# planck-epoch/unet-image-segmentation

Measured on AMD Instinct MI355X. Metric: images/sec (train step, 256x256x3), higher is better.
Workload: dtype f32; 1 GPU; configs[1]: 256x256x3 binary U-Net train step (fwd + dice_loss + bwd + AdamW + MeanIoU(2) update, dropout 0.2); network=U_NET separable-conv, filters 64-128-256-512, bneck 1024, global_batch=16, per_gpu_batch=16, seq_len=65536, parallelism=dp1, batchnorm=per-replica

## Files before the change

unet-image-segmentation_amd/csrc/gemm_wgrad.hip:

```cpp
#include "dispatch.h"
#include "gemm.h"

namespace unet {
namespace {

template <int BP, int BQ, int AMODE, bool ADROP, int BMODE, bool BDROP>
__global__ __launch_bounds__(256) void gemm_wgrad_kernel(WgradArgs g) {
    constexpr int LDA = BP + 4, LDB = BQ + 4;
    constexpr int TM = BP / 64, TN = BQ / 64;
    constexpr int AR = BP / 16, BR = BQ / 16;
    constexpr int AS = 256 / BP, BS = 256 / BQ;
    __shared__ float As[2][BK][LDA];
    __shared__ float Bs[2][BK][LDB];

    const int tid = threadIdx.x, lane = tid & 63, wave = tid >> 6;
    const int wp = wave >> 1, wq = wave & 1;
    const int lo = lane & 31, hi = lane >> 5;
    const int ntp = (g.P + BP - 1) / BP;
    const int p0 = (blockIdx.x % ntp) * BP;
    const int q0 = (blockIdx.x / ntp) * BQ;
    const int64_t mb = (int64_t)blockIdx.y * g.mslice;
    const int64_t me = mb + g.mslice < g.M ? mb + g.mslice : g.M;

    const int ap = tid % BP, amm = tid / BP;
    const int p = p0 + ap;
    const bool pv = p < g.P;
    float asc = 1.f, ash = 0.f;
    int poff = p;
    if constexpr (AMODE == W_BNRELU) {
        if (pv) {
            asc = g.a.sc0[p];
            ash = g.a.sh0[p];
        }
    }
    if constexpr (AMODE == W_UNSHUFFLE) {
        const int ab = p / g.uf;
        const int co = p - ab * g.uf;
        poff = (ab >> 1) * (2 * g.uW * g.uf) + (ab & 1) * g.uf + co;
    }
    const int bq = tid % BQ, bmm = tid / BQ;
    const int q = q0 + bq;
    const bool qv = q < g.Q;
    float bsc = 1.f, bsh = 0.f;
    if constexpr (BMODE == W_BNRELU) {
        if (qv) {
            bsc = g.b.sc0[q];
            bsh = g.b.sh0[q];
        }
    }

    float ra[AR], rb[BR];
    auto load_stage = [&](int64_t k0) {
#pragma unroll
        for (int r = 0; r < AR; ++r) {
            const int64_t m = k0 + amm + AS * r;
            float v = 0.f;
            if (pv && m < me) {
                if constexpr (AMODE == W_UNSHUFFLE) {
                    const int64_t hw = (int64_t)g.uH * g.uW;
                    const int n = (int)(m / hw);
                    const int rem = (int)(m - n * hw);
                    const int i = rem / g.uW, j = rem - (rem / g.uW) * g.uW;
                    v = g.a.src0[(int64_t)((n * 2 * g.uH + 2 * i) * 2 * g.uW + 2 * j) * g.uf + poff];
                } else {
                    v = g.a.src0[m * g.a.c0 + p];
                    if constexpr (AMODE == W_BNRELU) v = bnrelu(v, asc, ash);
                    if constexpr (ADROP) v *= drop_mult(g.a.seed, (uint64_t)m * g.a.C + p, g.a.rate, g.a.inv_keep);
                }
            }
            ra[r] = v;
        }
#pragma unroll
        for (int r = 0; r < BR; ++r) {
            const int64_t m = k0 + bmm + BS * r;
            float v = 0.f;
            if (qv && m < me) {
                v = g.b.src0[m * g.b.c0 + q];
                if constexpr (BMODE == W_BNRELU) v = bnrelu(v, bsc, bsh);
                if constexpr (BDROP) v *= drop_mult(g.b.seed, (uint64_t)m * g.b.C + q, g.b.rate, g.b.inv_keep);
            }
            rb[r] = v;
        }
    };
    auto store_stage = [&](int buf) {
#pragma unroll
        for (int r = 0; r < AR; ++r) As[buf][amm + AS * r][ap] = ra[r];
#pragma unroll
        for (int r = 0; r < BR; ++r) Bs[buf][bmm + BS * r][bq] = rb[r];
    };

    floatx16 acc[TM][TN];
#pragma unroll
    for (int tm = 0; tm < TM; ++tm)
#pragma unroll
        for (int tn = 0; tn < TN; ++tn)
#pragma unroll
            for (int r = 0; r < 16; ++r) acc[tm][tn][r] = 0.f;

    const int nk = (int)((me - mb + BK - 1) / BK);
    if (nk > 0) {
        load_stage(mb);
        store_stage(0);
    }
    __syncthreads();
    for (int kt = 0; kt < nk; ++kt) {
        const int buf = kt & 1;
        if (kt + 1 < nk) load_stage(mb + (int64_t)(kt + 1) * BK);
#pragma unroll
        for (int kk = 0; kk < BK / 2; ++kk) {
            float av[TM], bv[TN];
#pragma unroll
            for (int tm = 0; tm < TM; ++tm) av[tm] = As[buf][2 * kk + hi][wp * (BP / 2) + tm * 32 + lo];
#pragma unroll
            for (int tn = 0; tn < TN; ++tn) bv[tn] = Bs[buf][2 * kk + hi][wq * (BQ / 2) + tn * 32 + lo];
#pragma unroll
            for (int tm = 0; tm < TM; ++tm)
#pragma unroll
                for (int tn = 0; tn < TN; ++tn)
                    acc[tm][tn] = __builtin_amdgcn_mfma_f32_32x32x2f32(av[tm], bv[tn], acc[tm][tn], 0, 0, 0);
        }
        if (kt + 1 < nk) store_stage(buf ^ 1);
        __syncthreads();
    }
    float* slab = g.slab + (int64_t)blockIdx.y * g.P * g.Q;
#pragma unroll
    for (int tm = 0; tm < TM; ++tm)
#pragma unroll
        for (int tn = 0; tn < TN; ++tn) {
            const int qq = q0 + wq * (BQ / 2) + tn * 32 + lo;
            if (qq >= g.Q) continue;
#pragma unroll
            for (int r = 0; r < 16; ++r) {
                const int pp = p0 + wp * (BP / 2) + tm * 32 + acc_row(r, hi);
                if (pp < g.P) slab[(int64_t)pp * g.Q + qq] = acc[tm][tn][r];
            }
        }
}

template <int BP, int BQ, int AMODE, bool ADROP, int BMODE, bool BDROP>
__global__ __launch_bounds__(256, 1) void gemm_wgrad_vec(WgradArgs g) {
    constexpr int LDA = BP + 4, LDB = BQ + 4;
    constexpr int TM = BP / 64, TN = BQ / 64;
    constexpr int PQ = BP / 4, QQ = BQ / 4;
    constexpr int AR = BK * PQ / 256, BR = BK * QQ / 256;
    constexpr int AS = 256 / PQ, BS = 256 / QQ;
    __shared__ __attribute__((aligned(16))) char smem[4 * 2 * BK * (LDA + LDB)];
    float (*As)[BK * LDA] = reinterpret_cast<float (*)[BK * LDA]>(smem);
    float (*Bs)[BK * LDB] = reinterpret_cast<float (*)[BK * LDB]>(smem + 4 * 2 * BK * LDA);

    const int tid = threadIdx.x, lane = tid & 63, wave = tid >> 6;
    const int wp = wave >> 1, wq = wave & 1;
    const int lo = lane & 31, hi = lane >> 5;
    const int ntp = (g.P + BP - 1) / BP;
    int tile, slice;
    xcd_group_order_sx(gridDim.x, gridDim.y, tile, slice);
    const int p0 = (tile % ntp) * BP;
    const int q0 = (tile / ntp) * BQ;
    const int mb = (int)(slice * g.mslice);
    const int me = (int)((mb + g.mslice) < g.M ? (mb + g.mslice) : g.M);

    const int apq = tid % PQ, amm = tid / PQ;
    const int p = p0 + 4 * apq;
    const bool pv = p < g.P;
    float4 asc = f4(1.f), ash = f4(0.f);
    int poff = p;
    if constexpr (AMODE == W_BNRELU) {
        if (pv) {
            asc = ld4(g.a.sc0 + p);
            ash = ld4(g.a.sh0 + p);
        }
    }
    if constexpr (AMODE == W_UNSHUFFLE) {
        const int ab = p / g.uf;
        const int co = p - ab * g.uf;
        poff = (ab >> 1) * (2 * g.uW * g.uf) + (ab & 1) * g.uf + co;
    }
    const int bqq = tid % QQ, bmm = tid / QQ;
    const int q = q0 + 4 * bqq;
    const bool qv = q < g.Q;
    float4 bsc = f4(1.f), bsh = f4(0.f), bmu = f4(0.f), bp_ = f4(0.f), bq_ = f4(0.f);
    if constexpr (BMODE == W_BNRELU || BMODE == W_BNBWD) {
        if (qv) {
            bsc = ld4(g.b.sc0 + q);
            bsh = ld4(g.b.sh0 + q);
        }
    }
    if constexpr (BMODE == W_BNBWD) {
        if (qv) {
            bmu = ld4(g.bcoef + q);
            bp_ = ld4(g.bcoef + g.Q + q);
            bq_ = ld4(g.bcoef + 2 * g.Q + q);
        }
    }

    float4 ra[AR], rb[BR];
    int ur[AMODE == W_UNSHUFFLE ? AR : 1], uj[AMODE == W_UNSHUFFLE ? AR : 1];
    if constexpr (AMODE == W_UNSHUFFLE) {
#pragma unroll
        for (int r = 0; r < AR; ++r) {
            const int m = mb + amm + AS * r;
            ur[r] = m / g.uW;
            uj[r] = m - ur[r] * g.uW;
        }
    }
    auto load_stage = [&](int k0) {
#pragma unroll
        for (int r = 0; r < AR; ++r) {
            const int m = k0 + amm + AS * r;
            float4 v = f4(0.f);
            if (pv && m < me) {
                if constexpr (AMODE == W_UNSHUFFLE) {
                    v = ld4(g.a.src0 + (4 * ur[r] * g.uW + 2 * uj[r]) * g.uf + poff);
                } else {
                    v = ld4(g.a.src0 + (int64_t)m * g.a.c0 + p);
                    if constexpr (AMODE == W_BNRELU) v = bnrelu4(v, asc, ash);
                    if constexpr (ADROP) {
                        const uint64_t i = (uint64_t)m * g.a.C + p;
                        v = mul4(v, drop_mult4(g.a.seed, i, g.a.rate, g.a.inv_keep));
                    }
                }
            }
            ra[r] = v;
        }
#pragma unroll
        for (int r = 0; r < BR; ++r) {
            const int m = k0 + bmm + BS * r;
            float4 v = f4(0.f);
            if (qv && m < me) {
                v = ld4(g.b.src0 + (int64_t)m * g.b.c0 + q);
                if constexpr (BMODE == W_BNRELU) v = bnrelu4(v, bsc, bsh);
                if constexpr (BMODE == W_BNBWD)
                    bn_bwd_dz4(v, ld4(g.bz + (int64_t)m * g.b.c0 + q), bsc, bsh, bmu, bp_, bq_);
                if constexpr (BDROP) {
                    const uint64_t i = (uint64_t)m * g.b.C + q;
                    v = mul4(v, drop_mult4(g.b.seed, i, g.b.rate, g.b.inv_keep));
                }
            }
            rb[r] = v;
        }
        if constexpr (AMODE == W_UNSHUFFLE) {
#pragma unroll
            for (int r = 0; r < AR; ++r) {
                uj[r] += BK;
                while (uj[r] >= g.uW) {
                    uj[r] -= g.uW;
                    ++ur[r];
                }
            }
        }
    };
    const bool csum_on = g.colpart != nullptr && tile < ntp;
    float4 csum = f4(0.f);
    auto store_stage = [&](int buf) {
#pragma unroll
        for (int r = 0; r < AR; ++r) *reinterpret_cast<float4*>(&As[buf][(amm + AS * r) * LDA + 4 * apq]) = ra[r];
#pragma unroll
        for (int r = 0; r < BR; ++r) *reinterpret_cast<float4*>(&Bs[buf][(bmm + BS * r) * LDB + 4 * bqq]) = rb[r];
        if (csum_on) {
#pragma unroll
            for (int r = 0; r < AR; ++r) csum = add4(csum, ra[r]);
        }
    };

    floatx16 acc[TM][TN];
#pragma unroll
    for (int tm = 0; tm < TM; ++tm)
#pragma unroll
        for (int tn = 0; tn < TN; ++tn)
#pragma unroll
            for (int r = 0; r < 16; ++r) acc[tm][tn][r] = 0.f;

    const int nk = (me - mb + BK - 1) / BK;
    if (nk > 0) {
        load_stage(mb);
        store_stage(0);
    }
    __syncthreads();
    for (int kt = 0; kt < nk; ++kt) {
        const int buf = kt & 1;
        if (kt + 1 < nk) load_stage(mb + (kt + 1) * BK);
#pragma unroll
        for (int kk = 0; kk < BK / 2; ++kk) {
            float av[TM], bv[TN];
#pragma unroll
            for (int tm = 0; tm < TM; ++tm) av[tm] = As[buf][(2 * kk + hi) * LDA + wp * (BP / 2) + tm * 32 + lo];
#pragma unroll
            for (int tn = 0; tn < TN; ++tn) bv[tn] = Bs[buf][(2 * kk + hi) * LDB + wq * (BQ / 2) + tn * 32 + lo];
#pragma unroll
            for (int tm = 0; tm < TM; ++tm)
#pragma unroll
                for (int tn = 0; tn < TN; ++tn)
                    acc[tm][tn] = __builtin_amdgcn_mfma_f32_32x32x2f32(av[tm], bv[tn], acc[tm][tn], 0, 0, 0);
        }
        if (kt + 1 < nk) store_stage(buf ^ 1);
        __syncthreads();
    }
    if (csum_on) {
        float4* T = reinterpret_cast<float4*>(&As[0][0]);
        T[tid] = csum;
        __syncthreads();
        if (tid < PQ && pv) {
            float4 t = T[tid];
            for (int j = 1; j < AS; ++j) t = add4(t, T[j * PQ + tid]);
            st4(g.colpart + (int64_t)slice * g.P + p, t);
        }
    }
    float* slab = g.slab + (int64_t)slice * g.P * g.Q;
#pragma unroll
    for (int tm = 0; tm < TM; ++tm)
#pragma unroll
        for (int tn = 0; tn < TN; ++tn) {
            const int qq = q0 + wq * (BQ / 2) + tn * 32 + lo;
            if (qq >= g.Q) continue;
#pragma unroll
            for (int r = 0; r < 16; ++r) {
                const int pp = p0 + wp * (BP / 2) + tm * 32 + acc_row(r, hi);
                if (pp < g.P) slab[(int64_t)pp * g.Q + qq] = acc[tm][tn][r];
            }
        }
}

template <int AMODE, bool ADROP, int BMODE, bool BDROP>
void launch_wgrad_t(const WgradArgs& a, const WgradPlan& w, hipStream_t st) {
    dim3 grid((unsigned)w.tiles, (unsigned)w.S);
    const unsigned pad = (unsigned)lab_knob("UNET_WGRAD_LDSPAD", 0);
    const bool vec = a.P % 4 == 0 && a.Q % 4 == 0 && (AMODE != W_UNSHUFFLE || a.uf % 4 == 0) &&
                     (AMODE == W_UNSHUFFLE || a.a.c0 % 4 == 0) && a.b.c0 % 4 == 0 &&
                     ((uintptr_t)a.a.src0 | (uintptr_t)a.b.src0) % 16 == 0;
    const bool vk = vec || BMODE == W_BNBWD;
    with_int<128, 64>(w.bp, [&](auto BP) {
        with_int<128, 64>(w.bq, [&](auto BQ) {
            if (vk) gemm_wgrad_vec<BP(), BQ(), AMODE, ADROP, BMODE, BDROP><<<grid, 256, pad, st>>>(a);
            else if constexpr (BMODE != W_BNBWD)
                gemm_wgrad_kernel<BP(), BQ(), AMODE, ADROP, BMODE, BDROP><<<grid, 256, pad, st>>>(a);
        });
    });
}

}

int run_wgrad(WgradArgs a, int amode, int bmode, float* out, void* ws, size_t ws_bytes, hipStream_t st,
              const char* what) {
    WgradPlan w = wgrad_plan(a.M, a.P, a.Q);
    const size_t need = (size_t)w.S * a.P * a.Q * sizeof(float);
    UNET_CHECK_ARG(ws && ws_bytes >= need, "%s: workspace %zu < %zu", what, ws_bytes, need);
    a.mslice = w.mslice;
    a.slab = static_cast<float*>(ws);
    const bool ad = a.a.rate > 0.f, bd = a.b.rate > 0.f;
    if (amode == W_PLAIN && bmode == W_PLAIN) {
        launch_wgrad_t<W_PLAIN, false, W_PLAIN, false>(a, w, st);
    } else if (amode == W_UNSHUFFLE && (bmode == W_BNRELU || bmode == W_PLAIN)) {
        with_int<W_BNRELU, W_PLAIN>(bmode, [&](auto BM) {
            with_bool(bd, [&](auto BD) { launch_wgrad_t<W_UNSHUFFLE, false, BM(), BD()>(a, w, st); });
        });
    } else if (amode == W_BNRELU && bmode == W_PLAIN) {
        with_bool(ad, [&](auto AD) { launch_wgrad_t<W_BNRELU, AD(), W_PLAIN, false>(a, w, st); });
    } else {
        UNET_CHECK_ARG(false, "%s: unsupported wgrad operand modes %d/%d", what, amode, bmode);
    }
    UNET_CHECK_LAUNCH(what);
    return reduce_slabs(a.slab, w.S, (int64_t)a.P * a.Q, out, (int64_t)a.P * a.Q, (int64_t)a.P * a.Q, st);
}

size_t wgrad_workspace(int64_t M, int P, int Q) {
    WgradPlan w = wgrad_plan(M, P, Q);
    return align_up((size_t)w.S * P * Q * sizeof(float), 256);
}

int head_wgrad(const unet_view* x, int64_t M, const float* dlogit, int ncls, float* dkernel, void* ws, size_t ws_bytes,
               hipStream_t st) {
    WgradArgs a{};
    a.a = make_dview(*x);
    a.P = x->c0;
    a.b = plain_view(dlogit, ncls);
    a.Q = ncls;
    a.M = M;
    return run_wgrad(a, x->mode == UNET_VIEW_BNRELU ? W_BNRELU : W_PLAIN, W_PLAIN, dkernel, ws, ws_bytes, st,
                     "unet_head_bwd(filter)");
}
size_t head_wgrad_workspace(int64_t M, int cin, int ncls) { return wgrad_workspace(M, cin, ncls); }

}
```

Before: 1666 images/sec.

## Defer BN-ReLU and dropout transforms in wgrad to LDS store stage

For the vectorized weight-gradient GEMM with fused operand transforms, global loads now issue raw float4 values using 32-bit offsets from per-slice base pointers. The BN-ReLU scale/shift (cached in LDS), the dropout mask and the bounds masking are applied later in the store stage, after the MFMA loop. This moves address arithmetic and transform ALU work off the load path, so loads issue earlier and the transform math overlaps with outstanding memory traffic. It adds register-pressure tricks (asm barriers, sched_barrier) and a size check that rejects slices whose offsets would not fit in 32 bits.

```diff
diff --git a/unet-image-segmentation_amd/csrc/gemm_wgrad.hip b/unet-image-segmentation_amd/csrc/gemm_wgrad.hip
--- a/unet-image-segmentation_amd/csrc/gemm_wgrad.hip
+++ b/unet-image-segmentation_amd/csrc/gemm_wgrad.hip
@@ -137,6 +137,30 @@
         }
 }
 
+__device__ __forceinline__ unsigned drop_keep4(uint64_t seed, uint64_t idx, float rate) {
+    const uint64_t h = drop_hash(seed, idx >> 2);
+    unsigned keep = 0;
+#pragma unroll
+    for (int j = 0; j < 4; ++j) keep |= (drop_bit(h, j, rate, 1.f) != 0.f ? 1u : 0u) << j;
+    asm volatile("" : "+v"(keep));
+    return keep;
+}
+__device__ __forceinline__ float4 bnrelu4_halves(float4 v, const float* sc, const float* sh) {
+    const float2 s0 = *reinterpret_cast<const float2*>(sc), h0 = *reinterpret_cast<const float2*>(sh);
+    v.x = bnrelu(v.x, s0.x, h0.x);
+    v.y = bnrelu(v.y, s0.y, h0.y);
+    __builtin_amdgcn_sched_barrier(0);
+    const float2 s1 = *reinterpret_cast<const float2*>(sc + 2), h1 = *reinterpret_cast<const float2*>(sh + 2);
+    v.z = bnrelu(v.z, s1.x, h1.x);
+    v.w = bnrelu(v.w, s1.y, h1.y);
+    return v;
+}
+__device__ __forceinline__ float4 drop_apply4(float4 v, unsigned keep, float inv_keep) {
+    const int ik = __float_as_int(inv_keep);
+    auto mult = [&](int j) { return __int_as_float(ik & -(int)((keep >> j) & 1u)); };
+    return make_float4(v.x * mult(0), v.y * mult(1), v.z * mult(2), v.w * mult(3));
+}
+
 template <int BP, int BQ, int AMODE, bool ADROP, int BMODE, bool BDROP>
 __global__ __launch_bounds__(256, 1) void gemm_wgrad_vec(WgradArgs g) {
     constexpr int LDA = BP + 4, LDB = BQ + 4;
@@ -144,9 +168,13 @@
     constexpr int PQ = BP / 4, QQ = BQ / 4;
     constexpr int AR = BK * PQ / 256, BR = BK * QQ / 256;
     constexpr int AS = 256 / PQ, BS = 256 / QQ;
-    __shared__ __attribute__((aligned(16))) char smem[4 * 2 * BK * (LDA + LDB)];
+    constexpr bool LATE = !(AMODE == W_PLAIN && !ADROP && BMODE == W_PLAIN && !BDROP) && BMODE != W_BNBWD;
+    constexpr int NSS = LATE ? (AMODE == W_BNRELU ? 2 * BP : 0) + (BMODE == W_BNRELU ? 2 * BQ : 0) : 0;
+    __shared__ __attribute__((aligned(16))) char smem[4 * (2 * BK * (LDA + LDB) + NSS)];
     float (*As)[BK * LDA] = reinterpret_cast<float (*)[BK * LDA]>(smem);
     float (*Bs)[BK * LDB] = reinterpret_cast<float (*)[BK * LDB]>(smem + 4 * 2 * BK * LDA);
+    float* Ass = reinterpret_cast<float*>(smem + 4 * 2 * BK * (LDA + LDB));
+    float* Bss = Ass + (AMODE == W_BNRELU ? 2 * BP : 0);
 
     const int tid = threadIdx.x, lane = tid & 63, wave = tid >> 6;
     const int wp = wave >> 1, wq = wave & 1;
@@ -162,6 +190,7 @@
     const int apq = tid % PQ, amm = tid / PQ;
     const int p = p0 + 4 * apq;
     const bool pv = p < g.P;
+    const int pc = pv ? p : 0;
     float4 asc = f4(1.f), ash = f4(0.f);
     int poff = p;
     if constexpr (AMODE == W_BNRELU) {
@@ -169,10 +198,17 @@
             asc = ld4(g.a.sc0 + p);
             ash = ld4(g.a.sh0 + p);
         }
+        if constexpr (LATE) {
+            if (amm == 0) {
+                st4(Ass + 4 * apq, asc);
+                st4(Ass + BP + 4 * apq, ash);
+            }
+        }
     }
     if constexpr (AMODE == W_UNSHUFFLE) {
-        const int ab = p / g.uf;
-        const int co = p - ab * g.uf;
+        const int pu = LATE ? pc : p;
+        const int ab = pu / g.uf;
+        const int co = pu - ab * g.uf;
         poff = (ab >> 1) * (2 * g.uW * g.uf) + (ab & 1) * g.uf + co;
     }
     const int bqq = tid % QQ, bmm = tid / QQ;
@@ -185,6 +221,20 @@
             bsh = ld4(g.b.sh0 + q);
         }
     }
+    if constexpr (LATE && BMODE == W_BNRELU) {
+        if (bmm == 0) {
+            st4(Bss + 4 * bqq, bsc);
+            st4(Bss + BQ + 4 * bqq, bsh);
+        }
+    }
+    if constexpr (LATE && NSS > 0) __syncthreads();
+    int64_t aorg = (int64_t)mb * g.a.c0;
+    if constexpr (AMODE == W_UNSHUFFLE) {
+        const int r0 = mb / g.uW;
+        aorg = ((int64_t)4 * r0 * g.uW + 2 * (mb - r0 * g.uW)) * g.uf;
+    }
+    const char* abase = reinterpret_cast<const char*>(g.a.src0 + aorg);
+    const char* bbase = reinterpret_cast<const char*>(g.b.src0 + (int64_t)mb * g.b.c0);
     if constexpr (BMODE == W_BNBWD) {
         if (qv) {
             bmu = ld4(g.bcoef + q);
@@ -194,16 +244,59 @@
     }
 
     float4 ra[AR], rb[BR];
-    int ur[AMODE == W_UNSHUFFLE ? AR : 1], uj[AMODE == W_UNSHUFFLE ? AR : 1];
+    auto fresh = [](int v) {
+        asm volatile("" : "+v"(v));
+        return v;
+    };
+    constexpr int UR = AMODE == W_UNSHUFFLE ? (LATE ? 1 : AR) : 1;
+    int ur[UR], uj[UR];
     if constexpr (AMODE == W_UNSHUFFLE) {
 #pragma unroll
-        for (int r = 0; r < AR; ++r) {
+        for (int r = 0; r < UR; ++r) {
             const int m = mb + amm + AS * r;
             ur[r] = m / g.uW;
             uj[r] = m - ur[r] * g.uW;
+            if constexpr (LATE) {
+                const int r0 = mb / g.uW;
+                ur[r] = (4 * (ur[r] - r0) * g.uW + 2 * (uj[r] - (mb - r0 * g.uW))) * g.uf + poff;
+            }
         }
     }
     auto load_stage = [&](int k0) {
+        if constexpr (LATE) {
+            const int t = fresh(tid);
+            const int amm = t / PQ, bmm = t / QQ;
+            const int pc = p0 + 4 * (t % PQ) < g.P ? p0 + 4 * (t % PQ) : 0;
+            const int qc = q0 + 4 * (t % QQ) < g.Q ? q0 + 4 * (t % QQ) : 0;
+            unsigned ao[AR];
+            int oj = uj[0], oo = ur[0];
+#pragma unroll
+            for (int r = 0; r < AR; ++r) {
+                const int m = k0 + amm + AS * r;
+                if constexpr (AMODE == W_UNSHUFFLE) {
+                    if (r > 0) {
+                        oj += AS;
+                        oo += 2 * AS * g.uf;
+                        while (oj >= g.uW) {
+                            oj -= g.uW;
+                            oo += 2 * g.uW * g.uf;
+                        }
+                    }
+                    ao[r] = (unsigned)(m < me ? oo : 0);
+                } else {
+                    ao[r] = (unsigned)((m < me ? m - mb : 0) * g.a.c0 + pc);
+                }
+            }
+#pragma unroll
+            for (int r = 0; r < AR; ++r) ra[r] = ld4(reinterpret_cast<const float*>(abase + 4u * ao[r]));
+#pragma unroll
+            for (int r = 0; r < BR; ++r) {
+                const int m = k0 + bmm + BS * r;
+                const unsigned o = (unsigned)((m < me ? m - mb : 0) * g.b.c0 + qc);
+                rb[r] = ld4(reinterpret_cast<const float*>(bbase + 4u * o));
+            }
+            return;
+        }
 #pragma unroll
         for (int r = 0; r < AR; ++r) {
             const int m = k0 + amm + AS * r;
@@ -251,7 +344,65 @@
     };
     const bool csum_on = g.colpart != nullptr && tile < ntp;
     float4 csum = f4(0.f);
-    auto store_stage = [&](int buf) {
+    auto store_stage = [&](int buf, int k0) {
+        if constexpr (LATE) {
+            const int t = fresh(tid);
+            const int apq = t % PQ, amm = t / PQ, bqq = t % QQ, bmm = t / QQ;
+            const int p = p0 + 4 * apq, q = q0 + 4 * bqq;
+            const bool pv = p < g.P, qv = q < g.Q;
+#pragma unroll
+            for (int r = 0; r < AR; ++r) {
+                const int m = k0 + amm + AS * r;
+                float4 v = ra[r];
+                unsigned keep = 0;
+                if constexpr (ADROP) {
+                    keep = drop_keep4(g.a.seed, (uint64_t)m * g.a.C + p, g.a.rate);
+                    __builtin_amdgcn_sched_barrier(0);
+                }
+                if constexpr (AMODE == W_BNRELU) {
+                    if constexpr (ADROP) v = bnrelu4_halves(v, Ass + 4 * apq, Ass + BP + 4 * apq);
+                    else v = bnrelu4(v, ld4(Ass + 4 * apq), ld4(Ass + BP + 4 * apq));
+                }
+                if constexpr (ADROP) v = drop_apply4(v, keep, g.a.inv_keep);
+                v = pv && m < me ? v : f4(0.f);
+                *reinterpret_cast<float4*>(&As[buf][(amm + AS * r) * LDA + 4 * apq]) = v;
+                csum = add4(csum, v);
+                asm volatile("" : "+v"(csum.x), "+v"(csum.y), "+v"(csum.z), "+v"(csum.w));
+                __builtin_amdgcn_sched_barrier(0);
+            }
+            float4 sc = f4(1.f), sh = f4(0.f);
+            if constexpr (BMODE == W_BNRELU && !BDROP) {
+                sc = ld4(Bss + 4 * bqq);
+                sh = ld4(Bss + BQ + 4 * bqq);
+            }
+#pragma unroll
+            for (int r = 0; r < BR; ++r) {
+                const int m = k0 + bmm + BS * r;
+                float4 v = rb[r];
+                unsigned keep = 0;
+                if constexpr (BDROP) {
+                    keep = drop_keep4(g.b.seed, (uint64_t)m * g.b.C + q, g.b.rate);
+                    __builtin_amdgcn_sched_barrier(0);
+                }
+                if constexpr (BMODE == W_BNRELU) {
+                    if constexpr (BDROP) v = bnrelu4_halves(v, Bss + 4 * bqq, Bss + BQ + 4 * bqq);
+                    else v = bnrelu4(v, sc, sh);
+                }
+                if constexpr (BDROP) v = drop_apply4(v, keep, g.b.inv_keep);
+                v = qv && m < me ? v : f4(0.f);
+                *reinterpret_cast<float4*>(&Bs[buf][(bmm + BS * r) * LDB + 4 * bqq]) = v;
+                __builtin_amdgcn_sched_barrier(0);
+            }
+            if constexpr (AMODE == W_UNSHUFFLE) {
+                uj[0] += BK;
+                ur[0] += 2 * BK * g.uf;
+                while (uj[0] >= g.uW) {
+                    uj[0] -= g.uW;
+                    ur[0] += 2 * g.uW * g.uf;
+                }
+            }
+            return;
+        }
 #pragma unroll
         for (int r = 0; r < AR; ++r) *reinterpret_cast<float4*>(&As[buf][(amm + AS * r) * LDA + 4 * apq]) = ra[r];
 #pragma unroll
@@ -273,7 +424,7 @@
     const int nk = (me - mb + BK - 1) / BK;
     if (nk > 0) {
         load_stage(mb);
-        store_stage(0);
+        store_stage(0, mb);
     }
     __syncthreads();
     for (int kt = 0; kt < nk; ++kt) {
@@ -292,29 +443,36 @@
                 for (int tn = 0; tn < TN; ++tn)
                     acc[tm][tn] = __builtin_amdgcn_mfma_f32_32x32x2f32(av[tm], bv[tn], acc[tm][tn], 0, 0, 0);
         }
-        if (kt + 1 < nk) store_stage(buf ^ 1);
+        if (kt + 1 < nk) store_stage(buf ^ 1, mb + (kt + 1) * BK);
         __syncthreads();
     }
     if (csum_on) {
         float4* T = reinterpret_cast<float4*>(&As[0][0]);
+        int cp = p;
+        if constexpr (LATE) cp = p0 + 4 * (fresh(tid) % PQ);
         T[tid] = csum;
         __syncthreads();
-        if (tid < PQ && pv) {
+        if (tid < PQ && cp < g.P) {
             float4 t = T[tid];
             for (int j = 1; j < AS; ++j) t = add4(t, T[j * PQ + tid]);
-            st4(g.colpart + (int64_t)slice * g.P + p, t);
+            st4(g.colpart + (int64_t)slice * g.P + cp, t);
         }
     }
     float* slab = g.slab + (int64_t)slice * g.P * g.Q;
+    int elo = lo, ehi = hi, ewp = wp, ewq = wq;
+    if constexpr (LATE) {
+        const int t = fresh(tid);
+        elo = t & 31, ehi = (t >> 5) & 1, ewp = t >> 7, ewq = (t >> 6) & 1;
+    }
 #pragma unroll
     for (int tm = 0; tm < TM; ++tm)
 #pragma unroll
         for (int tn = 0; tn < TN; ++tn) {
-            const int qq = q0 + wq * (BQ / 2) + tn * 32 + lo;
+            const int qq = q0 + ewq * (BQ / 2) + tn * 32 + elo;
             if (qq >= g.Q) continue;
 #pragma unroll
             for (int r = 0; r < 16; ++r) {
-                const int pp = p0 + wp * (BP / 2) + tm * 32 + acc_row(r, hi);
+                const int pp = p0 + ewp * (BP / 2) + tm * 32 + acc_row(r, ehi);
                 if (pp < g.P) slab[(int64_t)pp * g.Q + qq] = acc[tm][tn][r];
             }
         }
@@ -346,6 +504,12 @@
     UNET_CHECK_ARG(ws && ws_bytes >= need, "%s: workspace %zu < %zu", what, ws_bytes, need);
     a.mslice = w.mslice;
     a.slab = static_cast<float*>(ws);
+    const int64_t rows = w.mslice + BK;
+    const int64_t ext_a = amode == W_UNSHUFFLE ? (rows + 2 * a.uW) * 4 * a.uf : rows * a.a.c0;
+    UNET_CHECK_ARG((amode == W_PLAIN && bmode == W_PLAIN && !(a.a.rate > 0.f) && !(a.b.rate > 0.f)) ||
+                       (ext_a < (int64_t(1) << 29) && rows * a.b.c0 < (int64_t(1) << 29)),
+                   "%s: a slice of %lld rows is too large for the viewed weight-gradient kernel", what,
+                   (long long)w.mslice);
     const bool ad = a.a.rate > 0.f, bd = a.b.rate > 0.f;
     if (amode == W_PLAIN && bmode == W_PLAIN) {
         launch_wgrad_t<W_PLAIN, false, W_PLAIN, false>(a, w, st);
```

Result: no change. 1679 images/sec (median of 6 runs) (+0.8%).
